# ZhengmaoHe/PARC

Measured on AMD Instinct MI355X. Metric: env-steps/sec (whole node), 4096 envs/GPU humanoid tracker at 1/2/4/8 MI355X, higher is better.
Workload: dtype f32; 1 GPU; 4096 envs/GPU tracker on procgen box heightfields, 64 synthetic clips (BASELINE.json configs[2]); envs_per_gpu=4096, env_steps_per_bench_step=131072, rollout_steps=32, update_epochs=5, minibatch=16384, sim_substeps=4, parallelism=dp1, scaling_rule=per-rank work fixed (T = 32, minibatch = 4 x envs): weak scaling, grad_allreduce=per minibatch (reference cadence)

## Files before the change

### include/parc_hip.h

```cpp
#ifndef PARC_HIP_H
#define PARC_HIP_H

#include <stdint.h>

#ifdef __cplusplus
extern "C" {
#endif

#define PARC_MAX_BODIES 16
#define PARC_MAX_DOFS 64
#define PARC_MAX_TAR_STEPS 6
#define PARC_MAX_KEY_BODIES 8

#define PARC_OK 0
#define PARC_EINVAL (-1)
#define PARC_EUNSUPPORTED (-2)

#define PARC_JOINT_ROOT 0
#define PARC_JOINT_HINGE 1
#define PARC_JOINT_SPHERICAL 2
#define PARC_JOINT_FIXED 3

#define PARC_DONE_NULL 0
#define PARC_DONE_FAIL 1
// ... 190 lines not shown

int64_t parc_sgd_workspace_floats(void);
int parc_sgd_momentum_step(void *stream, int64_t n, float *params, const float *grad, float *momentum_buf, float max_norm, float lr,
                           float momentum, float weight_decay, float *workspace, float *norm_out);

int parc_adamw_step(void *stream, int64_t n, float *params, const float *grad, float *exp_avg, float *exp_avg_sq, int64_t step,
                    float max_norm, float lr, float beta1, float beta2, float eps, float weight_decay, float *workspace, float *norm_out);

int parc_normalize_clamp(void *stream, int64_t rows, int dim, const float *x, const float *mean, const float *stdv, float clip, float *out);

int64_t parc_moments_workspace_floats(int64_t rows, int dim);
int parc_moments_accumulate(void *stream, int64_t rows, int dim, const float *x, float *acc, float *workspace);
int parc_obs_ingest(void *stream, int64_t rows, int dim, const float *x, const float *mean, const float *stdv, float clip, float *norm_out,
                    float *copy_dst, const int64_t *copy_row, float *acc, float *workspace);

int parc_action_head(void *stream, int n, int A, const float *mean, const float *logstd, const float *noise, const float *explore,
                     const float *a_mean, const float *a_std, float *action, float *logp);
int parc_action_head_record(void *stream, int n, int A, const float *mean, const float *logstd, const float *noise, const float *explore,
                            const float *a_mean, const float *a_std, float *action, float *logp, float *rec_action, float *rec_logp,
                            float *rec_mask, const float *forces_src, float *rec_forces, int n_forces, const int64_t *head);

int parc_points_hf_sdf(void *stream, int batch, int n_points, int dim_x, int dim_y, const float *points, const float *hf,
                       const float *min_box_center, const float *x_points, const float *y_points, float half_x, float half_y,
                       float base_z, int inverted, float radius, float *out, int32_t *out_cell);

int parc_points_hf_sdf_grad(void *stream, int batch, int n_points, int dim_x, int dim_y, const float *points, const float *hf,
                            const float *min_box_center, const float *x_points, const float *y_points, float half_x, float half_y,
                            float base_z, int inverted, const int32_t *cell, const float *g_out, float *g_points);

int64_t parc_relu_bwd_workspace_floats(int64_t rows, int dim);
int parc_relu_bwd_bias_grad(void *stream, int64_t rows, int dim, float *gy, const float *y, float *db, float *workspace);
int parc_weighted_colsum(void *stream, int64_t rows, int dim, const float *x, const float *w, float *out, float *workspace);

int parc_abi_version(void);

#ifdef __cplusplus
}
#endif
#endif
```

### parc_amd/_hip.py

```python
import ctypes
import os
import subprocess

import torch

_HERE = os.path.dirname(os.path.abspath(__file__))
LIB_DIR = os.path.join(_HERE, "lib")
LIB_PATH = os.path.join(LIB_DIR, "libparc_hip.so")
CSRC = os.path.join(_HERE, "csrc")
SOURCES = ["parc_kin.hip", "parc_sim.hip", "parc_ppo.hip", "parc_rollout.hip", "parc_optim.hip", "parc_colreduce.hip", "parc_terrain.hip", "parc_render.hip", "parc_score.hip", "parc_netstats.hip", "parc_moopt.hip",
           "parc_augment.hip", "parc_mdm_batch.hip", "parc_hfgather.hip", "parc_motion.hip", "parc_pose_opt.hip", "parc_returns.hip"]
DIAG_LIB_PATH = os.path.join(LIB_DIR, "libparc_hip_diag.so")
DIAG_SOURCES = SOURCES + ["parc_sim_ref.hip"]

MAX_BODIES = 16
MAX_DOFS = 64
MAX_TAR_STEPS = 6
MAX_KEY_BODIES = 8

POST_REF = 1
POST_OBS = 2
POST_REWARD_DONE = 4
POST_HF = 8
POST_MASKED = 16
# ... 170 lines not shown
    L.parc_update_fail_rates.argtypes = [c_vp, c_int, c_int, c_vp, c_vp, c_f, c_vp]
    L.parc_step_tail.argtypes = [c_vp, CharModelS, MotionLibS, EnvBuffersS, c_int, c_int, c_vp, c_f, c_vp]
    L.parc_step_tail.restype = c_int
    L.parc_td_lambda_return.argtypes = [c_vp, c_int, c_int, c_vp, c_vp, c_vp, c_f, c_f, c_vp]
    L.parc_adv_normalize.argtypes = [c_vp, c_int, c_vp, c_vp, c_vp, c_f, c_vp, c_vp, c_vp]
    L.parc_ppo_loss.argtypes = [c_vp, c_int, c_int] + [c_vp] * 8 + [PPOCfgS] + [c_vp] * 5
    L.parc_ppo_loss.restype = c_int
    L.parc_ppo_loss_packed.argtypes = [c_vp, c_int, c_int, c_vp, c_vp, c_vp, c_int, c_vp, PPOCfgS] + [c_vp] * 5
    L.parc_ppo_loss_packed.restype = c_int
    L.parc_ppo_workspace_floats.argtypes = [c_int]
    L.parc_ppo_workspace_floats.restype = c_int
    L.parc_normalize_clamp.argtypes = [c_vp, c_i64, c_int, c_vp, c_vp, c_vp, c_f, c_vp]
    L.parc_normalize_clamp.restype = c_int
    L.parc_action_head.argtypes = [c_vp, c_int, c_int] + [c_vp] * 8
    L.parc_action_head.restype = c_int
    L.parc_action_head_record.argtypes = [c_vp, c_int, c_int] + [c_vp] * 8 + [c_vp] * 5 + [c_int, c_vp]
    L.parc_action_head_record.restype = c_int
    L.parc_points_hf_sdf.argtypes = [c_vp, c_int, c_int, c_int, c_int] + [c_vp] * 5 + [c_f, c_f, c_f, c_int, c_f, c_vp, c_vp]
    L.parc_points_hf_sdf.restype = c_int
    L.parc_points_hf_sdf_grad.argtypes = [c_vp, c_int, c_int, c_int, c_int] + [c_vp] * 5 + [c_f, c_f, c_f, c_int, c_vp, c_vp, c_vp]
    L.parc_points_hf_sdf_grad.restype = c_int
    L.parc_scale_by_clipped_norm.argtypes = [c_vp, c_i64, c_vp, c_vp, c_f]
    L.parc_scale_by_clipped_norm.restype = c_int
    L.parc_moments_workspace_floats.argtypes = [c_i64, c_int]
    L.parc_moments_workspace_floats.restype = c_i64
    L.parc_moments_accumulate.argtypes = [c_vp, c_i64, c_int, c_vp, c_vp, c_vp]
    L.parc_moments_accumulate.restype = c_int
    L.parc_relu_bwd_workspace_floats.argtypes = [c_i64, c_int]
    L.parc_relu_bwd_workspace_floats.restype = c_i64
    L.parc_relu_bwd_bias_grad.argtypes = [c_vp, c_i64, c_int, c_vp, c_vp, c_vp, c_vp]
    L.parc_relu_bwd_bias_grad.restype = c_int
    L.parc_weighted_colsum.argtypes = [c_vp, c_i64, c_int, c_vp, c_vp, c_vp, c_vp]
    L.parc_weighted_colsum.restype = c_int
    L.parc_sgd_workspace_floats.argtypes = []
    L.parc_sgd_workspace_floats.restype = c_i64
    L.parc_sgd_momentum_step.argtypes = [c_vp, c_i64, c_vp, c_vp, c_vp, c_f, c_f, c_f, c_f, c_vp, c_vp]
    L.parc_sgd_momentum_step.restype = c_int
    L.parc_adamw_step.argtypes = [c_vp, c_i64, c_vp, c_vp, c_vp, c_vp, c_i64, c_f, c_f, c_f, c_f, c_f, c_f, c_vp, c_vp]
    L.parc_adamw_step.restype = c_int
    L.parc_return_tracker_update.argtypes = [c_vp, c_int, c_int, c_vp, c_i64] + [c_vp] * 8
    L.parc_return_tracker_workspace_floats.argtypes = [c_int]
    L.parc_return_tracker_workspace_floats.restype = c_i64
    L.parc_return_tracker_update.restype = c_int
    L.parc_record_step.argtypes = [c_vp, c_int, c_vp, c_int, c_vp]
    L.parc_record_step.restype = c_int
    L.parc_obs_ingest.argtypes = [c_vp, c_i64, c_int, c_vp, c_vp, c_vp, c_f, c_vp, c_vp, c_vp, c_vp, c_vp]
    L.parc_obs_ingest.restype = c_int
    L.parc_rng_step.argtypes = [c_vp, ctypes.c_uint64, c_vp, c_vp, c_i64, c_vp, c_i64, c_vp, c_int]
    L.parc_rng_step.restype = c_int
    L.parc_reset_apply.argtypes = [c_vp, c_int, c_vp, c_vp, c_vp, c_vp, c_vp, c_int] + [c_vp] * 9
    L.parc_reset_apply.restype = c_int
    L.parc_reset_sample_apply.argtypes = [c_vp, c_int, c_vp, c_vp, c_vp, c_int, c_vp, c_vp, c_f, c_vp, c_vp, c_int, c_f] + [c_vp] * 11
    L.parc_reset_sample_apply.restype = c_int
    for name in ("parc_refresh_ray_obs_hfs", "parc_refresh_obs_hfs", "parc_dof_to_rot", "parc_rot_to_dof",
                 "parc_forward_kinematics", "parc_calc_motion_frame", "parc_motion_lib_build", "parc_track_post_step", "parc_reset_apply",
                 "parc_update_fail_rates", "parc_td_lambda_return", "parc_adv_normalize"):
        getattr(L, name).restype = c_int
    if hasattr(L, "parc_sim_abi"):
        from . import _hip_sim
        _hip_sim.declare(L)
    if hasattr(L, "parc_render_abi"):
        from . import _hip_render
        _hip_render.declare(L)
    if hasattr(L, "parc_score_abi"):
        from . import _hip_score
        _hip_score.declare(L)
    if hasattr(L, "parc_netstats_abi"):
        from . import _hip_netstats
        _hip_netstats.declare(L)
    if hasattr(L, "parc_moopt_abi"):
        from . import _hip_moopt
        _hip_moopt.declare(L)
    if hasattr(L, "parc_augment_abi"):
        from . import _hip_augment
        _hip_augment.declare(L)
    if hasattr(L, "parc_mdm_batch_abi"):
        from . import _hip_mdm_batch
        _hip_mdm_batch.declare(L)


EXPORTED = ["parc_abi_version", "parc_refresh_ray_obs_hfs", "parc_refresh_obs_hfs", "parc_dof_to_rot", "parc_rot_to_dof",
            "parc_forward_kinematics", "parc_calc_motion_frame", "parc_motion_lib_build", "parc_track_post_step",
            "parc_update_fail_rates", "parc_td_lambda_return", "parc_adv_normalize", "parc_reset_apply", "parc_ppo_loss", "parc_ppo_workspace_floats", "parc_record_step", "parc_return_tracker_update", "parc_normalize_clamp",
            "parc_action_head", "parc_points_hf_sdf", "parc_moments_workspace_floats", "parc_moments_accumulate", "parc_reset_sample_apply", "parc_return_tracker_workspace_floats", "parc_scale_by_clipped_norm", "parc_relu_bwd_workspace_floats",
            "parc_relu_bwd_bias_grad", "parc_ppo_loss_packed", "parc_weighted_colsum", "parc_sgd_workspace_floats", "parc_sgd_momentum_step", "parc_adamw_step",
            "parc_pose_chain_forward", "parc_pose_chain_backward", "parc_points_hf_sdf_grad", "parc_body_points_world", "parc_body_points_world_grad",
            "parc_quat_diff_angle", "parc_quat_diff_angle_grad", "parc_temporal_terms", "parc_temporal_terms_grad", "parc_step_tail",
            "parc_assemble_obs", "parc_track_post_step_timed", "parc_rng_step", "parc_obs_ingest", "parc_action_head_record",
            "parc_render", "parc_render_abi", "parc_motion_score", "parc_score_abi",
            "parc_netstats_workspace_floats", "parc_netstats_update", "parc_netstats_abs_colsum", "parc_netstats_dormant_count", "parc_netstats_abi",
            "parc_points_hf_sdf_ragged", "parc_points_hf_sdf_ragged_grad", "parc_temporal_terms_seg", "parc_temporal_terms_seg_grad",
            "parc_segment_sums", "parc_moopt_abi",
            "parc_augment_frames", "parc_augment_terrains", "parc_augment_localize", "parc_augment_abi",
            "parc_mdm_heightfields", "parc_mdm_windows", "parc_mdm_batch_abi"]


def check(rc, what):
    if rc != 0:
        raise RuntimeError("{} failed with code {} ({})".format(what, rc, "bad argument" if rc == -1 else "unsupported" if rc == -2 else "hipError"))


def stream():
    return c_vp(torch.cuda.current_stream().cuda_stream)


def ptr(t):
    if t is None:
        return c_vp(0)
    assert t.is_cuda, "HIP kernels need device tensors (no CPU fallback)"
    assert t.is_contiguous(), "tensor must be contiguous"
    return c_vp(t.data_ptr())


def terrain_struct(hf, min_point, dxdy):
    assert hf.dtype == torch.float32 and hf.is_contiguous() and hf.dim() == 2
    return TerrainS(ptr(hf), int(hf.shape[0]), int(hf.shape[1]), float(min_point[0]), float(min_point[1]),
                    float(dxdy[0]), float(dxdy[1]))

# ... 28 lines not shown
```

### parc_amd/csrc/parc_colreduce.hip

```cpp
#include <hip/hip_runtime.h>
#include <stdint.h>

#include "../../include/parc_hip.h"
#include "parc_launch.h"
#include "parc_learner_math.h"

__global__ __launch_bounds__(256) void normalize_clamp_kernel(size_t n4, int dim4, const float4 *__restrict__ x, const float4 *__restrict__ mean,
                                                              const float4 *__restrict__ stdv, float clip, float4 *__restrict__ out) {
    for (size_t i = (size_t)blockIdx.x * blockDim.x + threadIdx.x; i < n4; i += (size_t)gridDim.x * blockDim.x) {
        const int c = (int)(i % (size_t)dim4);
        const float4 v = x[i], m = mean[c], s = stdv[c];
        float4 o;
        o.x = clamp_nan((v.x - m.x) / s.x, -clip, clip);
        o.y = clamp_nan((v.y - m.y) / s.y, -clip, clip);
        o.z = clamp_nan((v.z - m.z) / s.z, -clip, clip);
        o.w = clamp_nan((v.w - m.w) / s.w, -clip, clip);
        out[i] = o;
    }
}

extern "C" int parc_normalize_clamp(void *stream, int64_t rows, int dim, const float *x, const float *mean, const float *stdv, float clip,
                                    float *out) {
    if (rows < 0 || dim <= 0 || (dim & 3) || (((uintptr_t)x | (uintptr_t)mean | (uintptr_t)stdv | (uintptr_t)out) & 15)) return PARC_EINVAL;
    if (rows == 0) return PARC_OK;
// ... 141 lines not shown
    return PARC_OK;
}

#define RB_ROWS 128
__global__ __launch_bounds__(256) void relu_bwd_bias_partial_kernel(int rows, int dim4, float4 *__restrict__ gy, const float4 *__restrict__ y,
                                                                    float4 *__restrict__ partial) {
    __shared__ float4 red[4][64];
    const col_chunk_t k = col_chunk(rows, RB_ROWS);
    const int rg = k.rg, c = k.c, r0 = k.r0, r1 = k.r1;
    float4 s = make_float4(0.f, 0.f, 0.f, 0.f);
    if (c < dim4) {
#pragma unroll 4
        for (int r = r0 + rg; r < r1; r += 4) {
            const size_t i = (size_t)r * dim4 + c;
            float4 g = gy[i];
            const float4 a = y[i];
            g.x = a.x <= 0.f ? 0.f : g.x; g.y = a.y <= 0.f ? 0.f : g.y; g.z = a.z <= 0.f ? 0.f : g.z; g.w = a.w <= 0.f ? 0.f : g.w;
            gy[i] = g;
            s.x += g.x; s.y += g.y; s.z += g.z; s.w += g.w;
        }
    }
    fold_store(red, s, k, dim4, partial);
}

__global__ __launch_bounds__(256) void colsum_final_kernel(int chunks, int dim, const float *__restrict__ partial, float *__restrict__ out) {
    const int c = blockIdx.x * blockDim.x + threadIdx.x;
    if (c >= dim) return;
    float t = 0.f;
#pragma unroll 16
    for (int k = 0; k < chunks; ++k) t += partial[(size_t)k * dim + c];
    out[c] = t;
}

__global__ __launch_bounds__(256) void weighted_colsum_partial_kernel(int rows, int dim4, const float4 *__restrict__ x, const float *__restrict__ w,
                                                                      float4 *__restrict__ partial) {
    __shared__ float4 red[4][64];
    const col_chunk_t k = col_chunk(rows, RB_ROWS);
    const int rg = k.rg, c = k.c, r0 = k.r0, r1 = k.r1;
    float4 s = make_float4(0.f, 0.f, 0.f, 0.f);
    if (c < dim4) {
#pragma unroll 4
        for (int r = r0 + rg; r < r1; r += 4) {
            const float4 v = x[(size_t)r * dim4 + c];
            const float wr = w[r];
            s.x = fmaf(wr, v.x, s.x); s.y = fmaf(wr, v.y, s.y); s.z = fmaf(wr, v.z, s.z); s.w = fmaf(wr, v.w, s.w);
        }
    }
    fold_store(red, s, k, dim4, partial);
}

static void launch_colsum_final(void *stream, const col_grid_t &g, int dim, const float *workspace, float *out) {
    hipLaunchKernelGGL(colsum_final_kernel, dim3((dim + 255) / 256), dim3(256), 0, (hipStream_t)stream, g.chunks, dim, workspace, out);
}

extern "C" int parc_weighted_colsum(void *stream, int64_t rows, int dim, const float *x, const float *w, float *out, float *workspace) {
    const col_grid_t g = col_chunk_grid(rows, dim, RB_ROWS, (uintptr_t)x | (uintptr_t)workspace, !x || !w || !out || !workspace);
    if (g.rc != PARC_OK) return g.rc;
    if (rows > 0)
        hipLaunchKernelGGL(weighted_colsum_partial_kernel, g.grid, dim3(256), 0, (hipStream_t)stream, (int)rows, g.dim4, (const float4 *)x, w,
                           (float4 *)workspace);
    launch_colsum_final(stream, g, dim, workspace, out);
    PARC_CHECK_LAUNCH();
    return PARC_OK;
}

extern "C" int64_t parc_relu_bwd_workspace_floats(int64_t rows, int dim) {
    if (rows < 0 || dim <= 0) return -1;
    return ((rows + RB_ROWS - 1) / RB_ROWS) * (int64_t)dim;
}

extern "C" int parc_relu_bwd_bias_grad(void *stream, int64_t rows, int dim, float *gy, const float *y, float *db, float *workspace) {
    const col_grid_t g = col_chunk_grid(rows, dim, RB_ROWS, (uintptr_t)gy | (uintptr_t)y | (uintptr_t)workspace, !gy || !y || !db || !workspace);
    if (g.rc != PARC_OK) return g.rc;
    if (rows > 0)
        hipLaunchKernelGGL(relu_bwd_bias_partial_kernel, g.grid, dim3(256), 0, (hipStream_t)stream, (int)rows, g.dim4, (float4 *)gy, (const float4 *)y,
                           (float4 *)workspace);
    launch_colsum_final(stream, g, dim, workspace, db);
    PARC_CHECK_LAUNCH();
    return PARC_OK;
}
```

### parc_amd/learning/dm_ppo_agent.py

```python
import enum
import os
import time

import numpy as np
import torch

from ..envs import base_env
from ..gym_spaces import Box
from ..util import mp_util
from ..util.logger import Logger
from . import dm_ppo_model, experience_buffer, mp_optimizer, normalizer, rl_util, unit_stats
from .dm_ppo_return_tracker import DMPPOReturnTracker
from .tracking_error_tracker import TrackingErrorTracker


class AgentMode(enum.Enum):
    TRAIN = 0
    TEST = 1


_LOSS_KEYS = ["norm_obs", "action", "a_logp", "tar_val", "adv", "rand_action_mask"]


def enable_tuned_gemms():
# ... 456 lines not shown
            if torch.all(self._test_return_tracker.get_eps_per_env() > min_eps_per_env - 1):
                break
        out = {"mean_return": self._test_return_tracker.get_mean_return().item(),
               "mean_ep_len": self._test_return_tracker.get_mean_ep_len().item(),
               "num_eps": self._test_return_tracker.get_episodes()}
        if report_te:
            t = self._test_tracking_error_tracker
            out.update({"test_mean_root_pos_tracking_err": t.get_mean_root_pos_err().item(),
                        "test_mean_root_rot_tracking_err": t.get_mean_root_rot_err().item(),
                        "test_mean_body_pos_tracking_err": t.get_mean_body_pos_err().item(),
                        "test_mean_body_rot_tracking_err": t.get_mean_body_rot_err().item(),
                        "test_mean_dof_vel_tracking_err": t.get_mean_dof_vel_err().item(),
                        "test_mean_root_vel_tracking_err": t.get_mean_root_vel_err().item(),
                        "test_mean_root_ang_vel_tracking_err": t.get_mean_root_ang_vel_err().item()})
        return out

    def hard_reset_envs(self):
        if self._is_terrain_runner:
            self._env.apply_hard_reset()
        self._curr_obs, self._curr_info = self._env.reset()

    def test_model(self, num_episodes):
        self.eval()
        self.set_mode(AgentMode.TEST)
        self.hard_reset_envs()
        P = mp_util.get_num_procs()
        return self._rollout_test(int(np.ceil(num_episodes / P)))

    @torch.no_grad()
    def _critic_values(self):
        eb = self._exp_buffer
        obs, next_obs, done = eb.get_data("obs"), eb.get_data("next_obs"), eb.get_data("done")
        norm_obs = self._obs_norm.normalize(obs, out=eb.get_data("norm_obs"))
        vals = self._model.eval_critic(norm_obs).squeeze(-1)
        T = obs.shape[0]
        need = done != base_env.DoneFlags.NULL.value
        need[T - 1] = True
        next_vals = torch.empty_like(vals)
        next_vals[:T - 1] = vals[1:]
        idx = need.flatten().nonzero().flatten()
        sel = next_obs.flatten(0, 1)[idx]
        next_vals.flatten()[idx] = self._model.eval_critic(self._obs_norm.normalize(sel)).squeeze(-1)
        return vals, next_vals

    @torch.no_grad()
    def _build_train_data(self):
        self.eval()
        eb = self._exp_buffer
        obs, next_obs = eb.get_data("obs"), eb.get_data("next_obs")
        r, done = eb.get_data("reward"), eb.get_data("done")
        mask = eb.get_data("rand_action_mask")
        vals, next_vals = self._critic_values()
        r_min, r_max = self._env.get_reward_bounds()
        next_vals = torch.clamp(next_vals, r_min / (1.0 - self._discount), r_max / (1.0 - self._discount))
        succ_val = self._env.get_reward_succ() / (1.0 - self._discount)
        fail_val = self._env.get_reward_fail() / (1.0 - self._discount)
        next_vals = torch.where(done == base_env.DoneFlags.SUCC.value, torch.full_like(next_vals, succ_val), next_vals)
        next_vals = torch.where(done == base_env.DoneFlags.FAIL.value, torch.full_like(next_vals, fail_val), next_vals)
        new_vals = rl_util.compute_td_lambda_return(r, next_vals, done, self._discount, self._td_lambda)
        norm_adv, mean_std = rl_util.normalize_advantage(new_vals, vals, mask, self._norm_adv_clip)
        eb.set_data("tar_val", new_vals)
        eb.set_data("adv", norm_adv)
        if eb.has_buffer("loss_rec"):
            rec = eb.get_data("loss_rec")
            A = eb.get_data("action").shape[-1]
            self._a_norm.normalize(eb.get_data("action"), out=rec[..., 0:A])
            rec[..., A] = eb.get_data("a_logp")
            rec[..., A + 1] = norm_adv
            rec[..., A + 2] = mask
            rec[..., A + 3] = new_vals
        return {"adv_mean": mean_std[0], "adv_std": mean_std[1]}

    def _compute_loss(self, batch):
        norm_obs = batch["norm_obs"] if "norm_obs" in batch else self._obs_norm.normalize(batch["obs"])
        norm_a = self._a_norm.normalize(batch["action"])
# ... 38 lines not shown

    def _compute_loss_fused(self, batch, norm_obs, norm_a, pred):
        a_dist = self._model.eval_actor(norm_obs)
        logstd = a_dist.logstd
        if logstd.dim() != 2 or logstd.stride(0) != 0:
            return None
        loss, out = rl_util.ppo_loss(a_dist.mean, logstd[0], pred, norm_a, batch["a_logp"], batch["adv"], batch["rand_action_mask"],
                                     batch["tar_val"], self._ppo_clip_ratio, self._action_bound_weight, self._action_entropy_weight,
                                     self._action_reg_weight, self._critic_loss_weight, 20.0, self._critic_loss_type != "L2")
        slots = {"loss": 0, "critic_loss": 1, "actor_loss": 2, "clip_frac": 3, "imp_ratio": 4}
        if self._action_bound_weight != 0:
            slots["action_bound_loss"] = 5
        if self._action_entropy_weight != 0:
            slots["action_entropy"] = 6
        if self._action_reg_weight != 0:
            slots["action_reg_loss"] = 7
        return {"loss": loss, "_packed": out, "_slots": slots}

    def _explicit_update_ok(self):
        return (str(self._device).startswith("cuda") and self._config.get("explicit_backward", True) and self._config.get("fused_ppo_loss", True)
                and self._model.supports_explicit_backward())

    def _minibatch_step_explicit(self, batch, acc):
        norm_obs = batch["norm_obs"]
        mean, logstd, pred, saved = self._model.train_forward(norm_obs)
        if self._ppo_cfg is None:
            self._ppo_cfg = rl_util.ppo_cfg(self._ppo_clip_ratio, self._action_bound_weight, self._action_entropy_weight, self._action_reg_weight,
                                            self._critic_loss_weight, 20.0, self._critic_loss_type != "L2")
        if "loss_rec" in batch:
            out, g_mean, g_logstd, g_pred = rl_util.ppo_loss_and_grads_packed(mean, logstd, pred, batch["loss_rec"], self._ppo_cfg)
        else:
            out, g_mean, g_logstd, g_pred = rl_util.ppo_loss_and_grads(mean, logstd, pred, self._a_norm.normalize(batch["action"]), batch["a_logp"],
                                                                        batch["adv"], batch["rand_action_mask"], batch["tar_val"], self._ppo_cfg)
        write = lambda grad_of, done: self._model.train_backward(saved, g_mean, g_logstd, g_pred, grad_of, done)
        if self._clip_grad_norm:
            self._optimizer.step_explicit(write, model=self._model, max_norm=self._max_grad_norm)
        else:
            self._optimizer.step_explicit(write)
        acc.append(out)

    def _nan_trap(self, loss_rows, batches, epoch):
        bad = torch.isnan(loss_rows).any(dim=1).tolist()
        if not any(bad):
            return
        k = bad.index(True)
        import pickle
        batch_file = os.path.join("output", "debug_batch.pkl")
        os.makedirs("output", exist_ok=True)
        with open(batch_file, "wb") as f:
            pickle.dump({name: v.detach().cpu() for name, v in batches[k].items()}, f)
        Logger.print("NAN LOSS in minibatch {} of update epoch {}: wrote debug batch file to {}".format(k, epoch, batch_file))
        raise FloatingPointError("NaN loss in minibatch {} of update epoch {} (batch dumped to {}; the reference prints, dumps and exits "
                                 "at this point)".format(k, epoch, batch_file))

    def _update_model(self):
        self.train()
        N = self.get_num_envs()
        num_samples = self._exp_buffer.get_sample_count()
        batch_size = self._batch_size * N
        num_batches = int(np.ceil(float(num_samples) / batch_size))
        acc = dict()
        if self._explicit_update_ok():
            slots = {"loss": 0, "critic_loss": 1, "actor_loss": 2, "clip_frac": 3, "imp_ratio": 4}
            for name, w, i in (("action_bound_loss", self._action_bound_weight, 5), ("action_entropy", self._action_entropy_weight, 6),
                               ("action_reg_loss", self._action_reg_weight, 7)):
                if w != 0:
                    slots[name] = i
# ... 186 lines not shown
```

### parc_amd/learning/dm_ppo_model.py

```python
import enum

import numpy as np
import torch


class StdType(enum.Enum):
    FIXED = 0
    CONSTANT = 1
    VARIABLE = 2


class DistributionGaussianDiag:
    def __init__(self, mean, logstd):
        self._mean = mean
        self._logstd = logstd
        self._std_cache = None
        self._dim = mean.shape[-1]

    @property
    def _std(self):
        if self._std_cache is None:
            self._std_cache = torch.exp(self._logstd)
        return self._std_cache

# ... 126 lines not shown
        return self._action_dist(self._actor_layers(obs))

    @torch.no_grad()
    def eval_actor_tapped(self, obs):
        acts = self._trunk_forward(self._actor_layers, obs)
        mnet = self._action_dist._mean_net
        mean = torch.addmm(mnet.bias, acts[-1], mnet.weight.t())
        return DistributionGaussianDiag(mean=mean, logstd=torch.broadcast_to(self._action_dist._logstd_net, mean.shape)), acts[1:]

    def supports_explicit_backward(self):
        def plain(seq):
            mods = list(seq)
            return len(mods) % 2 == 0 and all(isinstance(m, torch.nn.Linear) for m in mods[0::2]) and all(isinstance(m, torch.nn.ReLU) for m in mods[1::2]) \
                and all(m.out_features % 4 == 0 for m in mods[0::2])
        return plain(self._actor_layers) and plain(self._critic_layers) and self._action_dist._std_type != StdType.VARIABLE

    @staticmethod
    def _trunk_forward(seq, x):
        acts = [x]
        for lin in list(seq)[0::2]:
            x = torch._addmm_activation(lin.bias, x, lin.weight.t(), use_gelu=False)
            acts.append(x)
        return acts

    @torch.no_grad()
    def train_forward(self, norm_obs):
        a = self._trunk_forward(self._actor_layers, norm_obs)
        c = self._trunk_forward(self._critic_layers, norm_obs)
        mnet = self._action_dist._mean_net
        mean = torch.addmm(mnet.bias, a[-1], mnet.weight.t())
        pred = torch.addmm(self._critic_out.bias, c[-1], self._critic_out.weight.t()).squeeze(-1)
        return mean, self._action_dist._logstd_net, pred, (a, c)

    def _relu_bwd(self, d, y, db):
        from .. import _hip
        L = _hip.lib()
        need = int(L.parc_relu_bwd_workspace_floats(d.shape[0], d.shape[1]))
        ws = getattr(self, "_relu_ws", None)
        if ws is None or ws.numel() < need or ws.device != d.device:
            ws = self._relu_ws = torch.empty(max(need, 1), dtype=torch.float32, device=d.device)
        _hip.check(L.parc_relu_bwd_bias_grad(_hip.stream(), d.shape[0], d.shape[1], _hip.ptr(d), _hip.ptr(y), _hip.ptr(db), _hip.ptr(ws)),
                   "parc_relu_bwd_bias_grad")

    def _weighted_colsum(self, x, w, out):
        from .. import _hip
        L = _hip.lib()
        need = int(L.parc_relu_bwd_workspace_floats(x.shape[0], x.shape[1]))
        ws = getattr(self, "_relu_ws", None)
        if ws is None or ws.numel() < need or ws.device != x.device:
            ws = self._relu_ws = torch.empty(max(need, 1), dtype=torch.float32, device=x.device)
        _hip.check(L.parc_weighted_colsum(_hip.stream(), x.shape[0], x.shape[1], _hip.ptr(x), _hip.ptr(w.contiguous()), _hip.ptr(out), _hip.ptr(ws)),
                   "parc_weighted_colsum")

    def _trunk_backward(self, seq, acts, d, grad_of, done):
        lins = list(seq)[0::2]
        for k in range(len(lins) - 1, -1, -1):
            lin = lins[k]
            self._relu_bwd(d, acts[k + 1], grad_of(lin.bias))
            torch.mm(d.t(), acts[k], out=grad_of(lin.weight))
            done(lin.weight)
            done(lin.bias)
            if k > 0:
                d = torch.mm(d, lin.weight)

    @torch.no_grad()
    def train_backward(self, saved, g_mean, g_logstd, g_pred, grad_of, done=lambda p: None):
        a, c = saved
        mnet = self._action_dist._mean_net
        torch.mm(g_mean.t(), a[-1], out=grad_of(mnet.weight))
        torch.sum(g_mean, dim=0, out=grad_of(mnet.bias))
        done(mnet.weight)
        done(mnet.bias)
        if self._action_dist._std_type == StdType.CONSTANT:
            grad_of(self._action_dist._logstd_net).copy_(g_logstd)
            done(self._action_dist._logstd_net)
        self._trunk_backward(self._actor_layers, a, torch.mm(g_mean, mnet.weight), grad_of, done)
        gp = g_pred.unsqueeze(-1)
        if self._critic_out.weight.shape[0] == 1:
            self._weighted_colsum(c[-1], g_pred, grad_of(self._critic_out.weight).view(-1))
        else:
            torch.mm(gp.t(), c[-1], out=grad_of(self._critic_out.weight))
        torch.sum(gp, dim=0, out=grad_of(self._critic_out.bias))
        done(self._critic_out.weight)
        done(self._critic_out.bias)
        self._trunk_backward(self._critic_layers, c, torch.mm(gp, self._critic_out.weight), grad_of, done)

    def eval_critic(self, obs):
        return self._critic_out(self._critic_layers(obs))
```

Measured before the change: 454,200 env-steps/s.

## Fuse PPO head backward into outer-colsum and dgrad-relu kernels; chunk critic eval

Adds custom HIP kernels for the small-output policy and critic heads. One computes the weight and bias gradients in a single column-reduction pass. The other fuses the input gradient, the ReLU mask and the last trunk bias gradient, replacing several GEMM, sum and relu-bwd launches. Critic value evaluation over the rollout buffer now runs in 16384-row chunks with addmm into a preallocated output, meant to cut peak memory and allocation traffic. This adds templated kernels and a bias sum done in fp64 partials, and GEMMs with thin shapes may run slower than rocBLAS.

```diff
diff --git a/include/parc_hip.h b/include/parc_hip.h
--- a/include/parc_hip.h
+++ b/include/parc_hip.h
@@ -246,6 +246,11 @@
 int parc_relu_bwd_bias_grad(void *stream, int64_t rows, int dim, float *gy, const float *y, float *db, float *workspace);
 int parc_weighted_colsum(void *stream, int64_t rows, int dim, const float *x, const float *w, float *out, float *workspace);
 
+int64_t parc_head_workspace_floats(int64_t rows, int dim, int A);
+int parc_outer_colsum(void *stream, int64_t rows, int dim, int A, const float *g, const float *x, float *dW, float *db, float *workspace);
+int parc_head_dgrad_relu(void *stream, int64_t rows, int dim, int A, const float *g, const float *W, const float *y, float *d, float *db,
+                         float *workspace);
+
 int parc_abi_version(void);
 
 #ifdef __cplusplus
diff --git a/parc_amd/_hip.py b/parc_amd/_hip.py
--- a/parc_amd/_hip.py
+++ b/parc_amd/_hip.py
@@ -226,6 +226,12 @@
     L.parc_relu_bwd_bias_grad.restype = c_int
     L.parc_weighted_colsum.argtypes = [c_vp, c_i64, c_int, c_vp, c_vp, c_vp, c_vp]
     L.parc_weighted_colsum.restype = c_int
+    L.parc_head_workspace_floats.argtypes = [c_i64, c_int, c_int]
+    L.parc_head_workspace_floats.restype = c_i64
+    L.parc_outer_colsum.argtypes = [c_vp, c_i64, c_int, c_int, c_vp, c_vp, c_vp, c_vp, c_vp]
+    L.parc_outer_colsum.restype = c_int
+    L.parc_head_dgrad_relu.argtypes = [c_vp, c_i64, c_int, c_int, c_vp, c_vp, c_vp, c_vp, c_vp, c_vp]
+    L.parc_head_dgrad_relu.restype = c_int
     L.parc_sgd_workspace_floats.argtypes = []
     L.parc_sgd_workspace_floats.restype = c_i64
     L.parc_sgd_momentum_step.argtypes = [c_vp, c_i64, c_vp, c_vp, c_vp, c_f, c_f, c_f, c_f, c_vp, c_vp]
@@ -277,7 +283,7 @@
             "parc_forward_kinematics", "parc_calc_motion_frame", "parc_motion_lib_build", "parc_track_post_step",
             "parc_update_fail_rates", "parc_td_lambda_return", "parc_adv_normalize", "parc_reset_apply", "parc_ppo_loss", "parc_ppo_workspace_floats", "parc_record_step", "parc_return_tracker_update", "parc_normalize_clamp",
             "parc_action_head", "parc_points_hf_sdf", "parc_moments_workspace_floats", "parc_moments_accumulate", "parc_reset_sample_apply", "parc_return_tracker_workspace_floats", "parc_scale_by_clipped_norm", "parc_relu_bwd_workspace_floats",
-            "parc_relu_bwd_bias_grad", "parc_ppo_loss_packed", "parc_weighted_colsum", "parc_sgd_workspace_floats", "parc_sgd_momentum_step", "parc_adamw_step",
+            "parc_relu_bwd_bias_grad", "parc_ppo_loss_packed", "parc_weighted_colsum", "parc_head_workspace_floats", "parc_outer_colsum", "parc_head_dgrad_relu", "parc_sgd_workspace_floats", "parc_sgd_momentum_step", "parc_adamw_step",
             "parc_pose_chain_forward", "parc_pose_chain_backward", "parc_points_hf_sdf_grad", "parc_body_points_world", "parc_body_points_world_grad",
             "parc_quat_diff_angle", "parc_quat_diff_angle_grad", "parc_temporal_terms", "parc_temporal_terms_grad", "parc_step_tail",
             "parc_assemble_obs", "parc_track_post_step_timed", "parc_rng_step", "parc_obs_ingest", "parc_action_head_record",
diff --git a/parc_amd/csrc/parc_colreduce.hip b/parc_amd/csrc/parc_colreduce.hip
--- a/parc_amd/csrc/parc_colreduce.hip
+++ b/parc_amd/csrc/parc_colreduce.hip
@@ -197,34 +197,230 @@
     out[c] = t;
 }
 
-__global__ __launch_bounds__(256) void weighted_colsum_partial_kernel(int rows, int dim4, const float4 *__restrict__ x, const float *__restrict__ w,
-                                                                      float4 *__restrict__ partial) {
+static void launch_colsum_final(void *stream, const col_grid_t &g, int dim, const float *workspace, float *out) {
+    hipLaunchKernelGGL(colsum_final_kernel, dim3((dim + 255) / 256), dim3(256), 0, (hipStream_t)stream, g.chunks, dim, workspace, out);
+}
+
+#define HEAD_MAX_A 32
+#define HEAD_ROWS_IN_FLIGHT(AT) ((AT) > 8 ? 8 : 16)
+#define HEAD_PIN2(t, o) "+v"(t[o]), "+v"(t[(o) + 1])
+#define HEAD_PIN4(t, o) HEAD_PIN2(t, o), HEAD_PIN2(t, (o) + 2)
+#define HEAD_PIN8(t, o) HEAD_PIN4(t, o), HEAD_PIN4(t, (o) + 4)
+#define HEAD_KEEP_LOADS_TOGETHER(N, t)                                                      \
+    do {                                                                                    \
+        static_assert(N == 2 || N == 4 || N == 8 || N == 16, "2, 4, 8 or 16 loaded values"); \
+        if constexpr (N == 2) asm volatile("" : HEAD_PIN2(t, 0));                            \
+        if constexpr (N == 4) asm volatile("" : HEAD_PIN4(t, 0));                            \
+        if constexpr (N == 8) asm volatile("" : HEAD_PIN8(t, 0));                            \
+        if constexpr (N == 16) asm volatile("" : HEAD_PIN8(t, 0), HEAD_PIN8(t, 8));          \
+    } while (0)
+
+template <int AT>
+__device__ __forceinline__ void stage_head_rows(float *__restrict__ gs, const float *__restrict__ g, int A, int r0, int r1) {
+    constexpr int PER = RB_ROWS * AT / 256;
+    const int n = (r1 - r0) * AT;
+    float t[PER];
+#pragma unroll
+    for (int j = 0; j < PER; ++j) {
+        const int i = threadIdx.x + 256 * j, rl = i / AT, a = i % AT;
+        t[j] = g[i < n && a < A ? (size_t)(r0 + rl) * A + a : (size_t)r0 * A];
+    }
+    HEAD_KEEP_LOADS_TOGETHER(PER, t);
+#pragma unroll
+    for (int j = 0; j < PER; ++j) {
+        const int i = threadIdx.x + 256 * j;
+        gs[i] = i < n && i % AT < A ? t[j] : 0.f;
+    }
+    __syncthreads();
+}
+
+template <int AT>
+__device__ __forceinline__ void fold_store_arrays(float4 (*red)[4][64], const float4 (&s)[AT], const col_chunk_t &k, int dim4, int A,
+                                                  float4 *__restrict__ row) {
+#pragma unroll
+    for (int b = 0; b < AT; b += 4) {
+        if (b) __syncthreads();
+#pragma unroll
+        for (int j = 0; j < 4; ++j)
+            if (b + j < AT) red[j][k.rg][k.lane] = s[b + j < AT ? b + j : 0];
+        __syncthreads();
+        if (b + k.rg < A && k.c < dim4) row[(size_t)(b + k.rg) * dim4 + k.c] = fold_row_groups(red[k.rg], k.lane);
+    }
+}
+
+template <int AT>
+__global__ __launch_bounds__(256, 1) void outer_colsum_partial_kernel(int rows, int dim4, int A, const float *__restrict__ g, const float4 *__restrict__ x,
+                                                                   float4 *__restrict__ partial, int width4, int want_db) {
+    __shared__ __attribute__((aligned(16))) float gs[RB_ROWS * AT];
+    __shared__ float4 red[AT < 4 ? AT : 4][4][64];
+    const col_chunk_t k = col_chunk(rows, RB_ROWS);
+    const int rg = k.rg, c = k.c, r0 = k.r0, r1 = k.r1;
+    if constexpr (AT > 1) stage_head_rows<AT>(gs, g, A, r0, r1);
+    float4 s[AT];
+#pragma unroll
+    for (int a = 0; a < AT; ++a) s[a] = make_float4(0.f, 0.f, 0.f, 0.f);
+    if (c < dim4) {
+        auto add_row = [&](int r, const float4 &v, float g1) {
+            const float *gr = AT > 1 ? gs + (r - r0) * AT : &g1;
+#pragma unroll
+            for (int a = 0; a < AT; ++a) {
+                const float w = gr[a];
+                s[a].x = fmaf(w, v.x, s[a].x); s[a].y = fmaf(w, v.y, s[a].y); s[a].z = fmaf(w, v.z, s[a].z); s[a].w = fmaf(w, v.w, s[a].w);
+            }
+        };
+        constexpr int U = HEAD_ROWS_IN_FLIGHT(AT);
+        int rb = r0 + rg;
+        for (; rb + 4 * (U - 1) < r1; rb += 4 * U) {
+            typedef float f32x4 __attribute__((ext_vector_type(4)));
+            f32x4 v[U];
+            float g1[U];
+#pragma unroll
+            for (int u = 0; u < U; ++u) {
+                v[u] = reinterpret_cast<const f32x4 *>(x)[(size_t)(rb + 4 * u) * dim4 + c];
+                g1[u] = AT == 1 ? g[rb + 4 * u] : 0.f;
+            }
+            HEAD_KEEP_LOADS_TOGETHER(U, v);
+#pragma unroll
+            for (int u = 0; u < U; ++u) add_row(rb + 4 * u, make_float4(v[u].x, v[u].y, v[u].z, v[u].w), g1[u]);
+        }
+        for (; rb < r1; rb += 4) add_row(rb, x[(size_t)rb * dim4 + c], AT == 1 ? g[rb] : 0.f);
+    }
+    float4 *row = partial + (size_t)blockIdx.y * width4;
+    fold_store_arrays<AT>(red, s, k, dim4, A, row);
+    if (!want_db || blockIdx.x != 0) return;
+    double sb = 0.0;
+    if (k.lane < AT)
+        for (int r = r0 + rg; r < r1; r += 4) sb += (double)(AT > 1 ? gs[(r - r0) * AT + k.lane] : g[r]);
+    __syncthreads();
+    double *redd = reinterpret_cast<double *>(red);
+    redd[rg * 64 + k.lane] = sb;
+    __syncthreads();
+    if (rg == 0 && k.lane < A)
+        reinterpret_cast<double *>(row + (size_t)A * dim4)[k.lane] = (redd[k.lane] + redd[64 + k.lane]) + (redd[128 + k.lane] + redd[192 + k.lane]);
+}
+
+__global__ __launch_bounds__(256) void outer_final_kernel(int chunks, int width, const float *__restrict__ partial, int n_w, float *__restrict__ dW,
+                                                          int n_b, float *__restrict__ db) {
+    __shared__ float red[4][64];
+    const int lane = threadIdx.x & 63, q = threadIdx.x >> 6;
+    if ((int)blockIdx.x < (n_w + 63) / 64) {
+        const int c = blockIdx.x * 64 + lane, per = (chunks + 3) / 4, k1 = min((q + 1) * per, chunks);
+        float t = 0.f;
+        if (c < n_w) {
+#pragma unroll 8
+            for (int k = q * per; k < k1; ++k) t += partial[(size_t)k * width + c];
+        }
+        red[q][lane] = t;
+        __syncthreads();
+        if (q == 0 && c < n_w) dW[c] = (red[0][lane] + red[1][lane]) + (red[2][lane] + red[3][lane]);
+        return;
+    }
+    for (int a = q; a < n_b; a += 4) {
+        double t = 0.0;
+        for (int k = lane; k < chunks; k += 64) t += reinterpret_cast<const double *>(partial + (size_t)k * width + n_w)[a];
+#pragma unroll
+        for (int o = 32; o >= 1; o >>= 1) t += __shfl_xor(t, o, 64);
+        if (lane == 0) db[a] = (float)t;
+    }
+}
+
+template <int AT>
+__global__ __launch_bounds__(256, 1) void head_dgrad_relu_partial_kernel(int rows, int dim4, int A, const float *__restrict__ g, const float *__restrict__ W,
+                                                                      const float4 *__restrict__ y, float4 *__restrict__ d, float4 *__restrict__ partial) {
+    __shared__ __attribute__((aligned(16))) float gs[RB_ROWS * AT];
     __shared__ float4 red[4][64];
     const col_chunk_t k = col_chunk(rows, RB_ROWS);
     const int rg = k.rg, c = k.c, r0 = k.r0, r1 = k.r1;
+    if constexpr (AT > 1) stage_head_rows<AT>(gs, g, A, r0, r1);
     float4 s = make_float4(0.f, 0.f, 0.f, 0.f);
     if (c < dim4) {
-#pragma unroll 4
-        for (int r = r0 + rg; r < r1; r += 4) {
-            const float4 v = x[(size_t)r * dim4 + c];
-            const float wr = w[r];
-            s.x = fmaf(wr, v.x, s.x); s.y = fmaf(wr, v.y, s.y); s.z = fmaf(wr, v.z, s.z); s.w = fmaf(wr, v.w, s.w);
-        }
+        float4 w[AT];
+#pragma unroll
+        for (int a = 0; a < AT; ++a) {
+            const float *wr = W + ((size_t)(a < A ? a : 0) * dim4 + c) * 4;
+            w[a] = a < A ? make_float4(wr[0], wr[1], wr[2], wr[3]) : make_float4(0.f, 0.f, 0.f, 0.f);
+        }
+        auto row_grad = [&](int r, const float4 &act, float g1) {
+            const float *gr = AT > 1 ? gs + (r - r0) * AT : &g1;
+            float4 v = make_float4(0.f, 0.f, 0.f, 0.f);
+#pragma unroll
+            for (int a = 0; a < AT; ++a) {
+                const float ga = gr[a];
+                v.x = fmaf(ga, w[a].x, v.x); v.y = fmaf(ga, w[a].y, v.y); v.z = fmaf(ga, w[a].z, v.z); v.w = fmaf(ga, w[a].w, v.w);
+            }
+            v.x = act.x <= 0.f ? 0.f : v.x; v.y = act.y <= 0.f ? 0.f : v.y; v.z = act.z <= 0.f ? 0.f : v.z; v.w = act.w <= 0.f ? 0.f : v.w;
+            d[(size_t)r * dim4 + c] = v;
+            s.x += v.x; s.y += v.y; s.z += v.z; s.w += v.w;
+        };
+        constexpr int U = HEAD_ROWS_IN_FLIGHT(AT);
+        int rb = r0 + rg;
+        for (; rb + 4 * (U - 1) < r1; rb += 4 * U) {
+            typedef float f32x4 __attribute__((ext_vector_type(4)));
+            f32x4 v[U];
+            float g1[U];
+#pragma unroll
+            for (int u = 0; u < U; ++u) {
+                v[u] = reinterpret_cast<const f32x4 *>(y)[(size_t)(rb + 4 * u) * dim4 + c];
+                g1[u] = AT == 1 ? g[rb + 4 * u] : 0.f;
+            }
+            HEAD_KEEP_LOADS_TOGETHER(U, v);
+#pragma unroll
+            for (int u = 0; u < U; ++u) row_grad(rb + 4 * u, make_float4(v[u].x, v[u].y, v[u].z, v[u].w), g1[u]);
+        }
+        for (; rb < r1; rb += 4) row_grad(rb, y[(size_t)rb * dim4 + c], AT == 1 ? g[rb] : 0.f);
     }
     fold_store(red, s, k, dim4, partial);
 }
 
-static void launch_colsum_final(void *stream, const col_grid_t &g, int dim, const float *workspace, float *out) {
-    hipLaunchKernelGGL(colsum_final_kernel, dim3((dim + 255) / 256), dim3(256), 0, (hipStream_t)stream, g.chunks, dim, workspace, out);
+static int head_tile(int A) { return A == 1 ? 1 : A <= 4 ? 4 : A <= 8 ? 8 : A <= 16 ? 16 : HEAD_MAX_A; }
+
+#define HEAD_TILE_SWITCH(A, LAUNCH) \
+    switch (head_tile(A)) {         \
+    case 1: LAUNCH(1); break;       \
+    case 4: LAUNCH(4); break;       \
+    case 8: LAUNCH(8); break;       \
+    case 16: LAUNCH(16); break;     \
+    default: LAUNCH(32); break;     \
+    }
+
+extern "C" int64_t parc_head_workspace_floats(int64_t rows, int dim, int A) {
+    if (rows < 0 || dim <= 0 || A <= 0) return -1;
+    return ((rows + RB_ROWS - 1) / RB_ROWS) * ((int64_t)A * dim + 2 * HEAD_MAX_A);
+}
+
+extern "C" int parc_outer_colsum(void *stream, int64_t rows, int dim, int A, const float *g, const float *x, float *dW, float *db, float *workspace) {
+    const col_grid_t cg = col_chunk_grid(rows, dim, RB_ROWS, (uintptr_t)x | (uintptr_t)workspace, A <= 0 || !g || !x || !dW || !workspace);
+    if (cg.rc != PARC_OK) return cg.rc;
+    if (A > HEAD_MAX_A || (int64_t)A * dim + 2 * HEAD_MAX_A > INT32_MAX) return PARC_EUNSUPPORTED;
+    const int n_w = A * dim, width = n_w + (db ? 2 * HEAD_MAX_A : 0);
+#define LAUNCH(AT)                                                                                                                              \
+    hipLaunchKernelGGL(outer_colsum_partial_kernel<AT>, cg.grid, dim3(256), 0, (hipStream_t)stream, (int)rows, cg.dim4, A, g, (const float4 *)x, \
+                       (float4 *)workspace, width / 4, db ? 1 : 0)
+    if (rows > 0) HEAD_TILE_SWITCH(A, LAUNCH)
+#undef LAUNCH
+    const int n_b = db ? A : 0;
+    hipLaunchKernelGGL(outer_final_kernel, dim3((n_w + 63) / 64 + (n_b ? 1 : 0)), dim3(256), 0, (hipStream_t)stream, cg.chunks, width,
+                       (const float *)workspace, n_w, dW, n_b, db);
+    PARC_CHECK_LAUNCH();
+    return PARC_OK;
 }
 
 extern "C" int parc_weighted_colsum(void *stream, int64_t rows, int dim, const float *x, const float *w, float *out, float *workspace) {
-    const col_grid_t g = col_chunk_grid(rows, dim, RB_ROWS, (uintptr_t)x | (uintptr_t)workspace, !x || !w || !out || !workspace);
-    if (g.rc != PARC_OK) return g.rc;
-    if (rows > 0)
-        hipLaunchKernelGGL(weighted_colsum_partial_kernel, g.grid, dim3(256), 0, (hipStream_t)stream, (int)rows, g.dim4, (const float4 *)x, w,
-                           (float4 *)workspace);
-    launch_colsum_final(stream, g, dim, workspace, out);
+    return parc_outer_colsum(stream, rows, dim, 1, w, x, out, nullptr, workspace);
+}
+
+extern "C" int parc_head_dgrad_relu(void *stream, int64_t rows, int dim, int A, const float *g, const float *W, const float *y, float *d, float *db,
+                                    float *workspace) {
+    const col_grid_t cg = col_chunk_grid(rows, dim, RB_ROWS, (uintptr_t)y | (uintptr_t)d | (uintptr_t)workspace,
+                                         A <= 0 || !g || !W || !y || !d || !db || !workspace);
+    if (cg.rc != PARC_OK) return cg.rc;
+    if (A > HEAD_MAX_A) return PARC_EUNSUPPORTED;
+#define LAUNCH(AT)                                                                                                                                 \
+    hipLaunchKernelGGL(head_dgrad_relu_partial_kernel<AT>, cg.grid, dim3(256), 0, (hipStream_t)stream, (int)rows, cg.dim4, A, g, W, (const float4 *)y, \
+                       (float4 *)d, (float4 *)workspace)
+    if (rows > 0) HEAD_TILE_SWITCH(A, LAUNCH)
+#undef LAUNCH
+    launch_colsum_final(stream, cg, dim, workspace, db);
     PARC_CHECK_LAUNCH();
     return PARC_OK;
 }
diff --git a/parc_amd/learning/dm_ppo_agent.py b/parc_amd/learning/dm_ppo_agent.py
--- a/parc_amd/learning/dm_ppo_agent.py
+++ b/parc_amd/learning/dm_ppo_agent.py
@@ -512,7 +512,10 @@
         eb = self._exp_buffer
         obs, next_obs, done = eb.get_data("obs"), eb.get_data("next_obs"), eb.get_data("done")
         norm_obs = self._obs_norm.normalize(obs, out=eb.get_data("norm_obs"))
-        vals = self._model.eval_critic(norm_obs).squeeze(-1)
+        chunked = norm_obs.is_cuda and norm_obs.dtype == torch.float32 and self._model.supports_explicit_backward()
+        critic = (lambda x: self._model.eval_critic_rows(x.flatten(0, -2)).view(x.shape[:-1])) if chunked \
+            else (lambda x: self._model.eval_critic(x).squeeze(-1))
+        vals = critic(norm_obs)
         T = obs.shape[0]
         need = done != base_env.DoneFlags.NULL.value
         need[T - 1] = True
@@ -520,7 +523,7 @@
         next_vals[:T - 1] = vals[1:]
         idx = need.flatten().nonzero().flatten()
         sel = next_obs.flatten(0, 1)[idx]
-        next_vals.flatten()[idx] = self._model.eval_critic(self._obs_norm.normalize(sel)).squeeze(-1)
+        next_vals.flatten()[idx] = critic(self._obs_norm.normalize(sel))
         return vals, next_vals
 
     @torch.no_grad()
@@ -625,7 +628,8 @@
         else:
             out, g_mean, g_logstd, g_pred = rl_util.ppo_loss_and_grads(mean, logstd, pred, self._a_norm.normalize(batch["action"]), batch["a_logp"],
                                                                         batch["adv"], batch["rand_action_mask"], batch["tar_val"], self._ppo_cfg)
-        write = lambda grad_of, done: self._model.train_backward(saved, g_mean, g_logstd, g_pred, grad_of, done)
+        write = lambda grad_of, done: self._model.train_backward(saved, g_mean, g_logstd, g_pred, grad_of, done,
+                                                                 head_kernels=self._config.get("head_kernels", True))
         if self._clip_grad_norm:
             self._optimizer.step_explicit(write, model=self._model, max_norm=self._max_grad_norm)
         else:
diff --git a/parc_amd/learning/dm_ppo_model.py b/parc_amd/learning/dm_ppo_model.py
--- a/parc_amd/learning/dm_ppo_model.py
+++ b/parc_amd/learning/dm_ppo_model.py
@@ -182,31 +182,54 @@
         pred = torch.addmm(self._critic_out.bias, c[-1], self._critic_out.weight.t()).squeeze(-1)
         return mean, self._action_dist._logstd_net, pred, (a, c)
 
+    def _colreduce_ws(self, need, device):
+        ws = getattr(self, "_relu_ws", None)
+        if ws is None or ws.numel() < need or ws.device != device:
+            ws = self._relu_ws = torch.empty(max(int(need), 1), dtype=torch.float32, device=device)
+        return ws
+
     def _relu_bwd(self, d, y, db):
         from .. import _hip
         L = _hip.lib()
-        need = int(L.parc_relu_bwd_workspace_floats(d.shape[0], d.shape[1]))
-        ws = getattr(self, "_relu_ws", None)
-        if ws is None or ws.numel() < need or ws.device != d.device:
-            ws = self._relu_ws = torch.empty(max(need, 1), dtype=torch.float32, device=d.device)
+        ws = self._colreduce_ws(L.parc_relu_bwd_workspace_floats(d.shape[0], d.shape[1]), d.device)
         _hip.check(L.parc_relu_bwd_bias_grad(_hip.stream(), d.shape[0], d.shape[1], _hip.ptr(d), _hip.ptr(y), _hip.ptr(db), _hip.ptr(ws)),
                    "parc_relu_bwd_bias_grad")
 
     def _weighted_colsum(self, x, w, out):
         from .. import _hip
         L = _hip.lib()
-        need = int(L.parc_relu_bwd_workspace_floats(x.shape[0], x.shape[1]))
-        ws = getattr(self, "_relu_ws", None)
-        if ws is None or ws.numel() < need or ws.device != x.device:
-            ws = self._relu_ws = torch.empty(max(need, 1), dtype=torch.float32, device=x.device)
+        ws = self._colreduce_ws(L.parc_relu_bwd_workspace_floats(x.shape[0], x.shape[1]), x.device)
         _hip.check(L.parc_weighted_colsum(_hip.stream(), x.shape[0], x.shape[1], _hip.ptr(x), _hip.ptr(w.contiguous()), _hip.ptr(out), _hip.ptr(ws)),
                    "parc_weighted_colsum")
 
-    def _trunk_backward(self, seq, acts, d, grad_of, done):
+    MAX_HEAD_OUTPUTS = 32
+
+    def _head_kernels_apply(self, seq, head, g):
+        return (g.is_cuda and g.dtype == torch.float32 and len(list(seq)) > 0 and head.weight.shape[0] <= self.MAX_HEAD_OUTPUTS
+                and head.weight.is_contiguous())
+
+    def _head_backward(self, head, g, h, last_bias, grad_of, done, after_head=lambda: None):
+        from .. import _hip
+        L = _hip.lib()
+        g = g.contiguous()
+        B, dim, A = h.shape[0], h.shape[1], g.shape[1]
+        ws = self._colreduce_ws(L.parc_head_workspace_floats(B, dim, A), h.device)
+        _hip.check(L.parc_outer_colsum(_hip.stream(), B, dim, A, _hip.ptr(g), _hip.ptr(h), _hip.ptr(grad_of(head.weight)), _hip.ptr(grad_of(head.bias)),
+                                       _hip.ptr(ws)), "parc_outer_colsum")
+        done(head.weight)
+        done(head.bias)
+        after_head()
+        d = torch.empty_like(h)
+        _hip.check(L.parc_head_dgrad_relu(_hip.stream(), B, dim, A, _hip.ptr(g), _hip.ptr(head.weight), _hip.ptr(h), _hip.ptr(d), _hip.ptr(grad_of(last_bias)),
+                                          _hip.ptr(ws)), "parc_head_dgrad_relu")
+        return d
+
+    def _trunk_backward(self, seq, acts, d, grad_of, done, masked=False):
         lins = list(seq)[0::2]
         for k in range(len(lins) - 1, -1, -1):
             lin = lins[k]
-            self._relu_bwd(d, acts[k + 1], grad_of(lin.bias))
+            if not (masked and k == len(lins) - 1):
+                self._relu_bwd(d, acts[k + 1], grad_of(lin.bias))
             torch.mm(d.t(), acts[k], out=grad_of(lin.weight))
             done(lin.weight)
             done(lin.bias)
@@ -214,18 +237,30 @@
                 d = torch.mm(d, lin.weight)
 
     @torch.no_grad()
-    def train_backward(self, saved, g_mean, g_logstd, g_pred, grad_of, done=lambda p: None):
+    def train_backward(self, saved, g_mean, g_logstd, g_pred, grad_of, done=lambda p: None, head_kernels=True):
         a, c = saved
         mnet = self._action_dist._mean_net
-        torch.mm(g_mean.t(), a[-1], out=grad_of(mnet.weight))
-        torch.sum(g_mean, dim=0, out=grad_of(mnet.bias))
-        done(mnet.weight)
-        done(mnet.bias)
-        if self._action_dist._std_type == StdType.CONSTANT:
-            grad_of(self._action_dist._logstd_net).copy_(g_logstd)
-            done(self._action_dist._logstd_net)
-        self._trunk_backward(self._actor_layers, a, torch.mm(g_mean, mnet.weight), grad_of, done)
+
+        def logstd_grad():
+            if self._action_dist._std_type == StdType.CONSTANT:
+                grad_of(self._action_dist._logstd_net).copy_(g_logstd)
+                done(self._action_dist._logstd_net)
+
+        if head_kernels and self._head_kernels_apply(self._actor_layers, mnet, g_mean):
+            d = self._head_backward(mnet, g_mean, a[-1], list(self._actor_layers)[-2].bias, grad_of, done, logstd_grad)
+            self._trunk_backward(self._actor_layers, a, d, grad_of, done, masked=True)
+        else:
+            torch.mm(g_mean.t(), a[-1], out=grad_of(mnet.weight))
+            torch.sum(g_mean, dim=0, out=grad_of(mnet.bias))
+            done(mnet.weight)
+            done(mnet.bias)
+            logstd_grad()
+            self._trunk_backward(self._actor_layers, a, torch.mm(g_mean, mnet.weight), grad_of, done)
         gp = g_pred.unsqueeze(-1)
+        if head_kernels and self._head_kernels_apply(self._critic_layers, self._critic_out, gp):
+            d = self._head_backward(self._critic_out, gp, c[-1], list(self._critic_layers)[-2].bias, grad_of, done)
+            self._trunk_backward(self._critic_layers, c, d, grad_of, done, masked=True)
+            return
         if self._critic_out.weight.shape[0] == 1:
             self._weighted_colsum(c[-1], g_pred, grad_of(self._critic_out.weight).view(-1))
         else:
@@ -237,3 +272,13 @@
 
     def eval_critic(self, obs):
         return self._critic_out(self._critic_layers(obs))
+
+    CRITIC_CHUNK_ROWS = 16384
+
+    @torch.no_grad()
+    def eval_critic_rows(self, x):
+        out = torch.empty(x.shape[0], dtype=x.dtype, device=x.device)
+        for s in range(0, x.shape[0], self.CRITIC_CHUNK_ROWS):
+            h = self._trunk_forward(self._critic_layers, x[s:s + self.CRITIC_CHUNK_ROWS])[-1]
+            torch.addmm(self._critic_out.bias, h, self._critic_out.weight.t(), out=out[s:s + h.shape[0]].unsqueeze(-1))
+        return out
```

After: 458,400 env-steps/s (median of 6 runs). About the same (+0.9%).
